# tbuckworth/train-procgen-pytorch

Hardware: AMD Instinct MI355X
Metric: env steps/sec (whole node), coinrun hard-500 IMPALA-CNN PPO (higher is better)
Workload: dtype bf16

## Files before the change

include/mi355ppo.h:

```cpp
#ifndef MI355PPO_H
#define MI355PPO_H
#include <stddef.h>
#include <stdint.h>
#ifdef __cplusplus
extern "C" {
#endif

typedef struct mi_ctx mi_ctx;

enum { MI_ARCH_IMPALA = 0, MI_ARCH_MLP = 1 };

typedef struct mi_config {
    int32_t arch;
    int32_t n_steps;
    int32_t n_envs;
    int32_t n_actions;
    int32_t obs_dim;
    int32_t mlp_depth;
    int32_t mlp_width;
    int32_t out_dim;
    int32_t max_batch;
    int32_t device;
    int32_t precision;
    int32_t value_from_logits;
// ... 20 lines not shown
int mi_copy_params(mi_ctx* dst, mi_ctx* src);
int mi_get_grads(mi_ctx* ctx, float* flat, int64_t n);
int mi_set_adam_state(mi_ctx* ctx, const float* exp_avg, const float* exp_avg_sq, int64_t n);
int mi_get_adam_state(mi_ctx* ctx, float* exp_avg, float* exp_avg_sq, int64_t n);

int mi_put_obs(mi_ctx* ctx, int32_t t, const void* obs, size_t bytes);
int mi_get_obs(mi_ctx* ctx, int32_t t, void* obs, size_t bytes);
int mi_put_step(mi_ctx* ctx, int32_t t, const float* rew, const float* done);
int mi_put_policy_outputs(mi_ctx* ctx, int32_t t, const int32_t* act, const float* logp, const float* value);
enum { MI_F_REW = 0, MI_F_DONE, MI_F_VALUE, MI_F_LOGP, MI_F_ADV, MI_F_RET, MI_F_ACT };
int mi_read_field(mi_ctx* ctx, int32_t field, float* out, int64_t n);
int mi_write_field(mi_ctx* ctx, int32_t field, const float* in, int64_t n);

int mi_policy_step(mi_ctx* ctx, int32_t t, uint64_t seed, const float* u,
                   int64_t* act_out, float* logp_out, float* value_out);

int mi_rollout_step(mi_ctx* ctx, int32_t t, const float* rew_prev, const float* done_prev, uint64_t seed, const float* u,
                    int64_t* act_out, float* logp_out, float* value_out);

int mi_rollout_groups(mi_ctx* ctx, int32_t n_groups);
int mi_rollout_submit(mi_ctx* ctx, int32_t t, int32_t group, const void* frames, size_t bytes, const float* rew_prev,
                      const float* done_prev, uint64_t seed, const float* u);
int mi_rollout_wait(mi_ctx* ctx, int32_t group, int64_t* act_out, float* logp_out, float* value_out);

int mi_predict_staged(mi_ctx* ctx, const void* obs, size_t bytes, uint64_t seed, uint64_t counter, const float* u,
                      int64_t* act_out, float* logp_out, float* value_out);
int mi_value_saliency(mi_ctx* ctx, const void* obs, size_t bytes, uint64_t seed, uint64_t counter, const float* u,
                      int64_t* act_out, float* logp_out, float* value_out, float* grad_out);
int mi_commit_staged(mi_ctx* ctx, int32_t t);

int mi_set_gru(mi_ctx* ctx, const float* w_ih, const float* w_hh, const float* b_ih, const float* b_hh);
int mi_rec_state(mi_ctx* ctx, const float* hidden , const float* done );
int mi_get_hidden(mi_ctx* ctx, float* hidden );
int mi_rec_begin(mi_ctx* ctx, const float* hidden , const float* done );
int mi_get_hidden_ring(mi_ctx* ctx, int32_t t0, int32_t t1, float* out );
int mi_forward_rec(mi_ctx* ctx, const void* obs, float* logp_all, float* value, float* hidden_out);

int mi_forward(mi_ctx* ctx, const void* obs, int32_t n, float* logp_all, float* value, float* feat);

int mi_compute_estimates(mi_ctx* ctx, float gamma, float lmbda, int32_t use_gae, int32_t normalize_adv);
int mi_adv_stats(mi_ctx* ctx, double stats3[3]);
int mi_adv_apply(mi_ctx* ctx, const double stats3[3]);

int mi_minibatch(mi_ctx* ctx, const int64_t* idx, int32_t n_idx, int32_t n_global, const mi_hparams* hp);
int mi_minibatch_multi(mi_ctx* ctx, const int64_t* idx, int32_t n_idx, const int32_t* seg_n, int32_t n_seg, int32_t n_global,
                       const mi_hparams* hp);
// ... 45 lines not shown
const char* mi_profile_class_name(int32_t class_id);

int mi_op_conv3x3(mi_ctx* ctx, int32_t mode , int32_t cin, int32_t cout, int32_t hw, int32_t n,
                  const void* in, int32_t in_is_u8, int32_t relu_in, const float* w_ref ,
                  const float* bias, const float* res, const float* mask, const float* dout,
                  float* out , float* dbias_out);
int mi_op_resblock(mi_ctx* ctx, int32_t mode, int32_t ch, int32_t hw, int32_t n, const float* x, const float* w1, const float* b1,
                   const float* w2, const float* b2, const float* a_fwd, const float* x_fwd, float* out_a, float* out_y);
int mi_op_maxpool(mi_ctx* ctx, int32_t mode , int32_t n, int32_t hw, int32_t c,
                  const float* in, const float* dout, float* out);
int mi_op_gemm(mi_ctx* ctx, int32_t M, int32_t N, int32_t K, const float* A, int64_t sam, int64_t sak,
               const float* B, int64_t sbk, int64_t sbn, float* C);
int mi_op_fc_bf16(mi_ctx* ctx, int32_t mode, int32_t n, int32_t D, const float* x, const float* W, const float* b, const float* dy,
                  float* out, float* out_b);
int mi_selftest_mfma(mi_ctx* ctx, float* max_err);
int mi_debug_read(mi_ctx* ctx, int32_t which, int32_t n, float* out);
int mi_debug_philox(mi_ctx* ctx, const uint32_t* ctr_key6, int32_t n, uint32_t* out4, float* u_out);
int mi_debug_gru_step(mi_ctx* ctx, int32_t n, int32_t H, const float* x, const float* h, const float* done, const float* w_ih,
                      const float* w_hh, const float* b_ih, const float* b_hh, float* h_out, float* h_copy);
int mi_debug_gru_seq(mi_ctx* ctx, int32_t T, int32_t n, int32_t H, const float* x, const float* h0, const float* mask, const float* w_ih,
                     const float* w_hh, const float* b_ih, const float* b_hh, const float* dOut, float* out_h, float* dX, float* dW_ih,
                     float* dW_hh, float* db_ih, float* db_hh);
int mi_debug_step_latency(mi_ctx* ctx, int32_t t, int32_t iters, int32_t mode, float* us_out);
int mi_debug_flags(mi_ctx* ctx, int32_t flags);

#ifdef __cplusplus
}
#endif
#endif
```

scratch/ro_timeline4.py:

```python
import csv, glob, sys, collections
f = glob.glob(sys.argv[1] + "/**/*kernel_trace.csv", recursive=True)[0]
rows = list(csv.DictReader(open(f)))
key = "Stream_Id" if "Stream_Id" in rows[0] else "Queue_Id"
by = collections.defaultdict(list)
for r in rows:
    by[r[key]].append(r)
streams = [(k, v) for k, v in by.items() if sum(1 for r in v if r["Kernel_Name"].startswith("heads_sample")) > 200]
print("streams with a rollout chain:", [(k, len(v)) for k, v in streams], "key", key)
k, v = streams[0]
v.sort(key=lambda r: int(r["Start_Timestamp"]))
idx = [i for i, r in enumerate(v) if r["Kernel_Name"].startswith("heads_sample")]
a, b = idx[-150], idx[-149]
base = int(v[a]["End_Timestamp"])
for r in v[a + 1:b + 1]:
    s, e = int(r["Start_Timestamp"]), int(r["End_Timestamp"])
    print(f"{(s - base) / 1e3:8.1f} us +{(e - s) / 1e3:7.1f}  {r['Kernel_Name'][:70]}")
dur, gap, cnt = collections.Counter(), collections.Counter(), collections.Counter()
for i in range(idx[-201] + 1, idx[-1] + 1):
    r, p = v[i], v[i - 1]
    n = r["Kernel_Name"][:40]
    dur[n] += (int(r["End_Timestamp"]) - int(r["Start_Timestamp"])) / 1e3
    gap[n] += (int(r["Start_Timestamp"]) - int(p["End_Timestamp"])) / 1e3
    cnt[n] += 1
print("kernel                                     n    avg_us   avg_gap_before_us")
for n in cnt:
    print(f"{n:40s} {cnt[n]:5d} {dur[n] / cnt[n]:8.1f} {gap[n] / cnt[n]:8.1f}")
print("step period us", (int(v[idx[-1]]["End_Timestamp"]) - int(v[idx[-201]]["End_Timestamp"])) / 200 / 1e3)
```

train-procgen-pytorch_amd/csrc/engine.hip:

```cpp
#include "engine_ctx.h"

thread_local std::string g_err;
thread_local hipStream_t tl_stream = nullptr;
thread_local float* tl_ws = nullptr;
thread_local size_t tl_ws_floats = 0;
const char* mi_last_error(void) { return g_err.c_str(); }

#define NCCLC(x)                                                                                         \
    do {                                                                                                 \
        ncclResult_t r_ = (x);                                                                           \
        if (r_ != ncclSuccess) return fail(-5, std::string(#x) + ": " + ncclGetErrorString(r_) + " @" + std::to_string(__LINE__)); \
    } while (0)

extern "C" int mi_comm_destroy(mi_ctx* c);
static void prof_harvest(mi_ctx* c);
static const char* kProfNames[PC_COUNT] = {
    "conv_fwd_3_16_64", "conv_fwd_16_16_32", "conv_fwd_16_32_32", "conv_fwd_32_32_16", "conv_fwd_32_32_8",
    "conv_dgrad_3_16_64(unused)", "conv_dgrad_16_16_32", "conv_dgrad_16_32_32", "conv_dgrad_32_32_16", "conv_dgrad_32_32_8",
    "conv_wgrad_3_16_64", "conv_wgrad_16_16_32", "conv_wgrad_16_32_32", "conv_wgrad_32_32_16", "conv_wgrad_32_32_8",
    "maxpool_fwd", "maxpool_bwd", "gemm", "slab_reduce",
    "resblock_fwd_(unused)", "resblock_fwd_16_16_32", "resblock_fwd_(unused)", "resblock_fwd_32_32_16", "resblock_fwd_32_32_8",
    "resblock_dgrad_(unused)", "resblock_dgrad_16_16_32", "resblock_dgrad_(unused)", "resblock_dgrad_32_32_16", "resblock_dgrad_32_32_8"};
struct GroupJob { int t; const void* frames; size_t bytes; bool pull; bool have_rd, last; const float* u; unsigned long long seed; unsigned ticket; };
struct GroupWorker {
    std::thread th; std::mutex mu; std::condition_variable cv;
    std::atomic<unsigned> posted{0}, done{0}; std::atomic<bool> sleeping{false}, quit{false};
    GroupJob job{}; int rc = 0; std::string err;
};

static inline char* obs_stage(mi_ctx* c) { return c->stage_frames ? (char*)c->stage_frames : (char*)c->stage_obs; }
struct GemmWs { float* p; size_t floats; };
static inline GemmWs gemm_ws(mi_ctx* c) { return tl_ws ? GemmWs{tl_ws, tl_ws_floats} : GemmWs{c->gemm_ws, c->gemm_ws_floats}; }
static hipStream_t side_stream(mi_ctx* c) {
    hipStream_t ss = (c->n_groups > 0 && c->gs[0]) ? c->gs[0] : c->side_stream;
    if (!ss) { hipStreamCreateWithFlags(&c->side_stream, hipStreamNonBlocking); ss = c->side_stream; }
    return ss;
}
static int64_t gru_count(const mi_ctx* c) { return 2 * (int64_t)3 * c->H * c->H + 2 * (int64_t)3 * c->H; }
struct GruTensor { float* p; size_t off, len; };
struct GruTensors { GruTensor t[4]; };
static inline GruTensors gru_tensors(mi_ctx* c) {
    const size_t H = c->H, W = 3 * H * H, B = 3 * H;
    return GruTensors{{{c->gru_wih, 0, W}, {c->gru_whh, W, W}, {c->gru_bih, 2 * W, B}, {c->gru_bhh, 2 * W + B, B}}};
}

static void add_tensor(mi_ctx* c, const std::string& name, int64_t n, int kind, int co, int ci, int64_t& ref, int64_t dev) {
    TensorDesc t{name, ref, dev, n, kind, co, ci};
    c->tensors.push_back(t);
    ref += n;
}

std::string net_err_take(mi_ctx* c) { std::lock_guard<std::mutex> lk(c->net_err_mu); std::string m; m.swap(c->net_err); return m; }
void net_err_set(mi_ctx* c, const std::string& m) { std::lock_guard<std::mutex> lk(c->net_err_mu); if (c->net_err.empty()) c->net_err = m; }

static void build_impala_layout(mi_ctx* c) {
// ... 86 lines not shown
}
static int download_flat(mi_ctx* c, const float* dbuf, float* flat, int64_t n) {
    ARG(n == c->n_params, "flat vector length != mi_param_count"); JOIN(c);
    std::vector<float> tmp(n);
    HIPC(hipMemcpyAsync(tmp.data(), dbuf, n * sizeof(float), hipMemcpyDeviceToHost, c->stream));
    HIPC(hipStreamSynchronize(c->stream));
    for (auto& t : c->tensors) to_ref_layout(t, tmp.data() + t.dev_off, flat + t.ref_off);
    return 0;
}

int mi_create(const mi_config* cfg, mi_ctx** out) {
    ARG(cfg && out, "null cfg/out");
    ARG(cfg->arch == MI_ARCH_IMPALA || cfg->arch == MI_ARCH_MLP, "arch");
    ARG(cfg->n_actions >= 1 && cfg->n_actions <= 16, "n_actions must be in [1,16]");
    ARG(cfg->n_steps >= 1 && cfg->n_envs >= 1 && cfg->max_batch >= 1, "n_steps/n_envs/max_batch");
    ARG(cfg->precision == 0 || cfg->precision == 1, "precision must be 0 (fp32) or 1 (bf16 activations)");
    ARG(cfg->value_from_logits == 0 || cfg->value_from_logits == 1, "value_from_logits must be 0 (fc_value head) or 1 (logsumexp of the logits)");
    if (cfg->arch == MI_ARCH_MLP) ARG(cfg->obs_dim >= 1 && cfg->mlp_depth >= 2 && cfg->mlp_width >= 1 && cfg->out_dim >= 1, "mlp dims");
    if (cfg->arch == MI_ARCH_IMPALA)
        ARG(cfg->out_dim == 0 || (cfg->out_dim >= 64 && cfg->out_dim <= 512 && cfg->out_dim % 64 == 0),
            "impala out_dim (output_dim) must be a multiple of 64 in [64, 512]");
    int ndev = 0;
    if (hipGetDeviceCount(&ndev) != hipSuccess || ndev == 0) return fail(-3, "no HIP device: the MI355X library has no CPU fallback");
    HIPC(hipSetDevice(cfg->device));
    mi_ctx* c = new mi_ctx();
    c->cfg = *cfg;
    c->T = cfg->n_steps; c->E = cfg->n_envs; c->A = cfg->n_actions;
    c->H = (cfg->arch == MI_ARCH_IMPALA && cfg->out_dim == 0) ? 256 : cfg->out_dim;
    c->NB = cfg->max_batch < cfg->n_envs ? cfg->n_envs : cfg->max_batch;
    c->bf = (cfg->arch == MI_ARCH_IMPALA) && cfg->precision == 1;
    c->lse = cfg->value_from_logits;
    c->es = c->bf ? 2.0 : 4.0;
    if (cfg->stream) { c->stream = (hipStream_t)cfg->stream; c->own_stream = false; }
    else { HIPC(hipStreamCreateWithFlags(&c->stream, hipStreamNonBlocking)); c->own_stream = true; }
    HIPC(hipEventCreateWithFlags(&c->ev_side_fork, hipEventDisableTiming)); HIPC(hipEventCreateWithFlags(&c->ev_side_join, hipEventDisableTiming));
    c->side_stream = nullptr; c->side_on = true; c->side.armed = false;
    if (cfg->arch == MI_ARCH_IMPALA) build_impala_layout(c); else build_mlp_layout(c);
    if (cfg->arch == MI_ARCH_IMPALA && !impala_regions_ok(c)) { delete c; return fail(-1, "internal: parameter layout does not split at embedder.fc.weight"); }

    const int64_t P = c->n_params, T = c->T, E = c->E, NB = c->NB;
    HIPC(dalloc(&c->params, P)); HIPC(dalloc(&c->grads, P)); HIPC(dalloc(&c->adam_m, P)); HIPC(dalloc(&c->adam_v, P));
    HIPC(dalloc(&c->rew, T * E)); HIPC(dalloc(&c->done, T * E)); HIPC(dalloc(&c->logp, T * E));
    HIPC(dalloc(&c->adv, T * E)); HIPC(dalloc(&c->ret, T * E)); HIPC(dalloc(&c->value, (T + 1) * E));
    HIPC(dalloc(&c->act, T * E)); HIPC(dalloc(&c->adv_stats, 4));
    c->frames = nullptr; c->obsf = nullptr; c->stage_frames = nullptr; c->stage_obs = nullptr;
    if (cfg->arch == MI_ARCH_IMPALA) {
// ... 107 lines not shown
    }
    c->gru_x = c->gru_dg = nullptr; c->sal_keep_x = c->bwd_from_dfeat = false;
    c->gru_on = false; c->gru_wih = c->gru_whh = c->gru_bih = c->gru_bhh = c->h_state = c->h_masked = c->gru_gi = c->gru_gh = c->d_done = nullptr;
    c->h_ring = c->h_rec_stage = nullptr; c->ev_rec = nullptr; for (bool& b : c->g_rec_ok) b = false;
    c->gru_train = c->rec_last = false; c->gru_g = c->gru_m = c->gru_v = nullptr; c->gru_sumsq = nullptr;
    c->rec_x = c->rec_gi = c->rec_sv = c->rec_dgi = c->rec_dgh = c->rec_hm = c->rec_mask = c->rec_h0 = nullptr;
    HIPC(hipDeviceSynchronize());
    *out = c;
    return 0;
}

int mi_destroy(mi_ctx* c) {
    if (!c) return 0;
    mi_comm_destroy(c);
    for (int g = 0; g < mi_ctx::MAX_GROUPS; ++g)
        if (c->gw[g]) {
            GroupWorker* w = c->gw[g];
            w->quit.store(true); { std::lock_guard<std::mutex> lk(w->mu); } w->cv.notify_one();
            w->th.join(); delete w; c->gw[g] = nullptr;
        }
    for (int g = 0; g < mi_ctx::MAX_GROUPS; ++g) if (c->gs[g]) hipStreamSynchronize(c->gs[g]);
    prof_harvest(c);
    hipStreamSynchronize(c->stream);
    for (int g = 0; g < mi_ctx::MAX_GROUPS; ++g) if (c->gs[g]) { hipStreamDestroy(c->gs[g]); hipEventDestroy(c->ev_fork[g]); hipEventDestroy(c->ev_join[g]); }
    for (hipEvent_t e : c->prof.pool) hipEventDestroy(e);
    float* fl[] = {c->params, c->grads, c->adam_m, c->adam_v, c->rew, c->done, c->logp, c->adv, c->ret, c->value, c->obsf,
                   c->feat, c->dfeat, c->hout, c->dY, c->GC, c->GP[0], c->GP[1], c->GP[2], c->slabs, c->gemm_ws, c->col_ws,
                   c->fs_scratch, c->fs_val, c->lut, c->stage_obs, c->loss_partial, c->loss_stats, c->loss_log, c->gnorm,
                   c->d_u, c->d_lp};
    for (float* p : fl) if (p) hipFree(p);
    if (c->cfg.arch == MI_ARCH_IMPALA)
        for (int b = 0; b < 3; ++b) { Block& k = c->blk[b]; hipFree(k.C); hipFree(k.PI); hipFree(k.P0); hipFree(k.A1); hipFree(k.P1); hipFree(k.A2); hipFree(k.P2); }
    for (float* p : c->mlp_act) if (p) hipFree(p);
    if (c->frames) hipFree(c->frames);
    if (c->stage_frames) hipFree(c->stage_frames);
    hipFree(c->s_act); hipFree(c->s_logp); hipFree(c->s_val);
    if (c->d_val) hipFree(c->d_val);
    if (c->fc_wp) hipFree(c->fc_wp); if (c->fc_wt) hipFree(c->fc_wt);
    if (c->banks) hipFree(c->banks); if (c->d_bank_desc) hipFree(c->d_bank_desc); if (c->c1_bank) hipFree(c->c1_bank);
    hipFree(c->stats_ring); hipFree(c->fs_ring); hipFree(c->fs_parts); if (c->d_slab_desc) hipFree(c->d_slab_desc); if (c->sal_dc) hipFree(c->sal_dc); if (c->sal_dx) hipFree(c->sal_dx); hipFree(c->d_pack); hipFree(c->d_rd); hipHostFree(c->h_pack); hipHostFree(c->h_rd); hipFree(c->d_done_ctr); if (c->side_stream) hipStreamDestroy(c->side_stream); hipEventDestroy(c->ev_side_fork); hipEventDestroy(c->ev_side_join); hipHostFree(c->h_flag);
    { float* gr[] = {c->gru_wih, c->gru_whh, c->gru_bih, c->gru_bhh, c->h_state, c->h_masked, c->gru_gi, c->gru_gh, c->d_done, c->gru_x, c->gru_dg}; for (float* q : gr) if (q) hipFree(q); }
    if (c->h_ring) hipFree(c->h_ring); if (c->h_rec_stage) hipHostFree(c->h_rec_stage); if (c->ev_rec) hipEventDestroy(c->ev_rec);
    { float* gt[] = {c->gru_g, c->gru_m, c->gru_v, c->rec_x, c->rec_gi, c->rec_sv, c->rec_dgi, c->rec_dgh, c->rec_hm, c->rec_mask, c->rec_h0}; for (float* q : gt) if (q) hipFree(q); }
    if (c->gru_sumsq) hipFree(c->gru_sumsq);
    hipFree(c->act); hipFree(c->adv_stats); hipFree(c->d_idx); hipFree(c->sumsq);
    if (c->fs_colmax) hipFree(c->fs_colmax); if (c->fs_arg) hipFree(c->fs_arg);
    if (c->fs_keys) hipFree(c->fs_keys); if (c->fs_keys_local) hipFree(c->fs_keys_local); if (c->d_gpos) hipFree(c->d_gpos); if (c->h_gpos) hipHostFree(c->h_gpos);
// ... 739 lines not shown
        while (w->posted.load(std::memory_order_acquire) == seen && !w->quit.load()) {
            if (++spins < 40000) __builtin_ia32_pause();
            else {
                std::unique_lock<std::mutex> lk(w->mu);
                w->sleeping.store(true);
                w->cv.wait_for(lk, std::chrono::milliseconds(50), [&] { return w->posted.load() != seen || w->quit.load(); });
                w->sleeping.store(false);
                spins = 0;
            }
        }
        if (w->quit.load()) return;
        seen = w->posted.load(std::memory_order_acquire);
        w->rc = group_issue(c, g, w->job);
        if (w->rc) w->err = g_err;
        w->done.store(seen, std::memory_order_release);
    }
}

int mi_rollout_groups(mi_ctx* c, int32_t n_groups) {
    ARG(c, "null"); ARG(n_groups >= 1 && n_groups <= mi_ctx::MAX_GROUPS, "1 .. 4 groups");
    ARG(c->E % n_groups == 0, "n_envs must be divisible by the number of groups");
    for (int g = 0; g < c->n_groups; ++g) ARG(!c->g_busy[g], "a group step is still in flight: mi_rollout_wait it first");
    JOIN(c);
    for (int g = 0; g < n_groups; ++g)
        if (!c->gs[g]) {
            HIPC(hipStreamCreateWithFlags(&c->gs[g], hipStreamNonBlocking));
            HIPC(hipEventCreateWithFlags(&c->ev_fork[g], hipEventDisableTiming));
            HIPC(hipEventCreateWithFlags(&c->ev_join[g], hipEventDisableTiming));
            c->gw[g] = new GroupWorker();
            c->gw[g]->th = std::thread(group_worker_main, c, g);
        }
    c->n_groups = n_groups;
    return 0;
}

int mi_rollout_submit(mi_ctx* c, int32_t t, int32_t g, const void* frames, size_t bytes, const float* rew_prev, const float* done_prev,
                      uint64_t seed, const float* u) {
    ARG(c, "null"); ARG(t >= 0 && t <= c->T, "t out of range"); ARG(g >= 0 && g < c->n_groups, "group out of range");
    ARG(c->gs[g], "call mi_rollout_groups first"); ARG(!c->g_busy[g], "this group's previous step has not been waited for");
    ARG(c->pending_n < 0, "a multirank minibatch is pending");
    const int E = c->E, ng = E / c->n_groups, e0 = g * ng;
    ARG(!frames || bytes == (size_t)ng * c->obs_bytes_per_env, "frames byte count != (E / groups) * bytes_per_env");
    if (rew_prev || done_prev) ARG(rew_prev && done_prev && t >= 1, "rew_prev/done_prev come together and belong to step t-1");
    if (c->gru_on) {
        ARG(c->h_ring && (t > 0 || c->g_rec_ok[g]), "recurrent rollout: call mi_rec_begin before the groups' first step (t == 0) of every rollout");
        if (t == 0) c->g_rec_ok[g] = false;
    }
    GroupWorker* w = c->gw[g];
    worker_drain(w);
    if (!c->g_forked[g]) {
        fc_refresh(c);
        HIPC(hipEventRecord(c->ev_fork[g], c->main_stream));
        HIPC(hipStreamWaitEvent(c->gs[g], c->ev_fork[g], 0));
        c->g_forked[g] = true;
    }
// ... 605 lines not shown
```

train-procgen-pytorch_amd/csrc/engine_ctx.h:

```cpp
#pragma once
#include "common.h"
#include "../../include/mi355ppo.h"
#include <rccl/rccl.h>
#include <math.h>
#include <stdio.h>
#include <string.h>
#include <string>
#include <unordered_map>
#include <vector>
#include <atomic>
#include <chrono>
#include <condition_variable>
#include <mutex>
#include <thread>

#pragma clang diagnostic ignored "-Wc++20-designator"
#define MI_INTERNAL __attribute__((visibility("hidden")))

MI_INTERNAL extern thread_local std::string g_err;
MI_INTERNAL extern thread_local hipStream_t tl_stream;
MI_INTERNAL extern thread_local float* tl_ws;
MI_INTERNAL extern thread_local size_t tl_ws_floats;
#define CUR(c) (tl_stream ? tl_stream : (c)->stream)
static inline int fail(int code, const std::string& msg) { g_err = msg; return code; }
// ... 69 lines not shown
    unsigned short* lut16;
    uint8_t* stage_frames; float* stage_obs;
    int32_t* d_idx;
    float *loss_partial, *loss_stats, *loss_log; int log_count, log_cap;
    double* fs_parts;
    float *stats_ring, *fs_ring; LossArgs ring_args;
    double* sumsq; float* gnorm;
    float* d_u; float* d_lp;
    unsigned short* banks; BankDesc* d_bank_desc; int n_banks;
    unsigned short* c1_bank;
    unsigned short *fc_wp, *fc_wt;
    bool fc_packed_valid;
    float *d_pack, *h_pack, *h_rd, *d_rd;
    unsigned *d_done_ctr, *h_flag, roll_ticket;
    int32_t* s_act; float *s_logp, *s_val; bool staged_valid;
    bool gru_on; float *gru_wih, *gru_whh, *gru_bih, *gru_bhh, *h_state, *h_masked, *gru_gi, *gru_gh, *d_done;
    float *gru_x, *gru_dg; bool sal_keep_x, bwd_from_dfeat;
    static constexpr int IDX_RING = 32;
    int32_t* h_idx_ring[IDX_RING]; hipEvent_t idx_ev[IDX_RING]; bool idx_used[IDX_RING]; int idx_next, idx_ev_deferred;
    float* h_f; int32_t* h_i; size_t h_f_floats;
    int multirank;
    LossArgs pending; int pending_n;
    static constexpr int MAX_GROUPS = 4;
    int n_groups; hipStream_t main_stream, gs[MAX_GROUPS]; hipEvent_t ev_fork[MAX_GROUPS], ev_join[MAX_GROUPS];
    bool g_forked[MAX_GROUPS], g_busy[MAX_GROUPS], g_last[MAX_GROUPS], g_dirty[MAX_GROUPS]; unsigned g_ticket[MAX_GROUPS]; bool groups_live;
    struct GroupWorker* gw[MAX_GROUPS];
    std::atomic<int64_t> copy_slot_ns{0}; double copy_rate_bytes_per_us;
    std::unordered_map<const void*, bool> pull_ok; bool no_pull;
    hipStream_t side_stream; hipEvent_t ev_side_fork, ev_side_join;
    bool side_on;
    struct SideJob { bool armed; LossArgs a; SegTab st; int mode; float* ring; float* fsr; float* log; } side;
    bool rollout_tail;
    float *fs_colmax, fs_grad_coef; int *fs_arg, fs_G;
    long long *fs_keys, *fs_keys_local; int32_t *d_gpos, *h_gpos; int gpos_n; bool fs_global_pending, fs_global_apply;
    ncclComm_t comm, comm_grad; int comm_world, comm_rank; hipStream_t comm_stream; hipEvent_t ev_ar_ready, ev_ar_done;
    bool ar_armed, ar_issued, ar_inflight; double* adv_all;
    std::string net_err; std::mutex net_err_mu;
    float *h_ring, *h_rec_stage; hipEvent_t ev_rec; bool g_rec_ok[MAX_GROUPS];
    bool gru_train, rec_last; float *gru_g, *gru_m, *gru_v; double* gru_sumsq;
    float *rec_x, *rec_gi, *rec_sv, *rec_dgi, *rec_dgh, *rec_hm, *rec_mask, *rec_h0;
};

static inline char* obs_ring(mi_ctx* c) { return c->frames ? (char*)c->frames : (char*)c->obsf; }

MI_INTERNAL std::string net_err_take(mi_ctx* c);
MI_INTERNAL void net_err_set(mi_ctx* c, const std::string& m);
MI_INTERNAL int join_groups(mi_ctx* c);
// ... 18 lines not shown
```

train-procgen-pytorch_amd/csrc/engine_ops.hip:

```cpp
#include "engine_ctx.h"

static int shape_of(int cin, int cout, int hw, ConvShape* s) {
    for (int k = 0; k < CS_COUNT; ++k) {
        int a, b, h; conv_shape_dims((ConvShape)k, &a, &b, &h);
        if (a == cin && b == cout && h == hw) { *s = (ConvShape)k; return 0; }
    }
    return fail(-1, "unsupported conv shape");
}

std::vector<uint16_t> host_to_bf16(const float* x, size_t n) {
    std::vector<uint16_t> o(n);
    for (size_t k = 0; k < n; ++k) { uint32_t u; memcpy(&u, x + k, 4); o[k] = (uint16_t)((u + 0x7FFFu + ((u >> 16) & 1u)) >> 16); }
    return o;
}
static void host_from_bf16(const uint16_t* h, float* x, size_t n) {
    for (size_t k = 0; k < n; ++k) { const uint32_t u = ((uint32_t)h[k]) << 16; memcpy(x + k, &u, 4); }
}
struct OpMem {
    static constexpr size_t GUARD = 64 * 1024;
    static constexpr int CANARY = 0xA5;
    struct Band { std::string name; unsigned char* p; size_t bytes; bool rezero; };
    const char* hook; hipStream_t st;
    std::vector<void*> owned;
    std::vector<Band> bands;
// ... 352 lines not shown
    HIPC(hipStreamSynchronize(c->stream));
    hipGraph_t graph = nullptr; hipGraphExec_t exec = nullptr;
    if (mode == 1) {
        HIPC(hipStreamBeginCapture(c->stream, hipStreamCaptureModeThreadLocal));
        issue();
        HIPC(hipStreamEndCapture(c->stream, &graph));
        HIPC(hipGraphInstantiate(&exec, graph, nullptr, nullptr, 0));
        HIPC(hipGraphLaunch(exec, c->stream)); HIPC(hipStreamSynchronize(c->stream));
    }
    const auto t0 = std::chrono::steady_clock::now();
    for (int k = 0; k < iters; ++k) {
        if (mode == 1) HIPC(hipGraphLaunch(exec, c->stream)); else issue();
        HIPC(hipStreamSynchronize(c->stream));
    }
    const auto t1 = std::chrono::steady_clock::now();
    *us_out = (float)(std::chrono::duration_cast<std::chrono::nanoseconds>(t1 - t0).count() / 1e3 / iters);
    if (exec) hipGraphExecDestroy(exec);
    if (graph) hipGraphDestroy(graph);
    c->prof.on = prof_on;
    HIPC(hipGetLastError()); NETCHK(c);
    return 0;
}

int mi_debug_read(mi_ctx* c, int32_t which, int32_t n, float* out) {
    ARG(c && out, "null"); JOIN(c); ARG(n >= 1 && n <= c->NB, "n must be in [1, max_batch]");
    if (which == 100 || which == 101 || which == 102) {
        ARG(which == 100 || c->rec_last, "which = 101 / 102: only after mi_minibatch_rec");
        const float* srcp = which == 102 ? c->dfeat : (which == 100 && c->rec_last) ? c->rec_x : c->feat;
        HIPC(hipMemcpyAsync(out, srcp, (size_t)n * c->H * 4, hipMemcpyDeviceToHost, c->stream));
        HIPC(hipStreamSynchronize(c->stream));
        return 0;
    }
    ARG(c->cfg.arch == MI_ARCH_IMPALA && which >= 0 && which < 24 && (which & 7) <= 5, "which");
    const Block& k = c->blk[which >> 3];
    const size_t pe = (size_t)n * (k.hin / 2) * (k.hin / 2) * k.cout;
    HIPC(hipStreamSynchronize(c->stream));
    if ((which & 7) == 5) {
        std::vector<uint8_t> h(pe);
        HIPC(hipMemcpy(h.data(), k.PI, pe, hipMemcpyDeviceToHost));
        for (size_t i = 0; i < pe; ++i) out[i] = (float)h[i];
        return 0;
    }
    const float* src[5] = {k.P0, k.A1, k.P1, k.A2, k.P2};
    return download_act(c, src[which & 7], out, pe);
}

// ... 117 lines not shown
```

train-procgen-pytorch_amd/mi355/engine.py:

```python
import ctypes as C
import os

import numpy as np

_HERE = os.path.dirname(os.path.abspath(__file__))
_LIB = None

ARCH_IMPALA, ARCH_MLP = 0, 1
F_REW, F_DONE, F_VALUE, F_LOGP, F_ADV, F_RET, F_ACT = range(7)
PTR_GRADS, PTR_LOSS_STATS, PTR_PARAMS, PTR_STATS_RING, PTR_FS_KEYS = 0, 1, 2, 3, 4
LOSS_FIELDS = ("pi_loss", "value_loss", "entropy", "x_ent", "total", "fs", "marg", "_pad")


class EngineError(RuntimeError):
    pass


class _Config(C.Structure):
    _fields_ = [("arch", C.c_int32), ("n_steps", C.c_int32), ("n_envs", C.c_int32), ("n_actions", C.c_int32),
                ("obs_dim", C.c_int32), ("mlp_depth", C.c_int32), ("mlp_width", C.c_int32), ("out_dim", C.c_int32),
                ("max_batch", C.c_int32), ("device", C.c_int32), ("precision", C.c_int32), ("value_from_logits", C.c_int32),
                ("reserved", C.c_int32 * 4),
                ("stream", C.c_void_p)]


class _HParams(C.Structure):
    _fields_ = [(n, C.c_float) for n in ("eps_clip", "value_coef", "entropy_coef", "x_entropy_coef",
                                         "entropy_multiplier", "fs_coef")]


def lib_path():
    return os.path.join(_HERE, "libmi355ppo.so")


EXPORTS = ("mi_last_error mi_create mi_destroy mi_sync mi_host_alloc mi_host_free mi_host_register mi_host_unregister mi_param_count mi_set_params "
           "mi_get_params mi_copy_params mi_get_grads mi_set_adam_state mi_get_adam_state mi_put_obs mi_get_obs mi_put_step "
           "mi_put_policy_outputs mi_read_field mi_write_field mi_policy_step mi_rollout_step mi_rollout_groups mi_rollout_submit mi_rollout_wait mi_predict_staged mi_value_saliency mi_commit_staged mi_set_gru mi_rec_state mi_get_hidden mi_rec_begin mi_get_hidden_ring mi_forward_rec mi_forward mi_compute_estimates "
           "mi_adv_stats mi_adv_apply mi_minibatch mi_minibatch_multi mi_optimizer_step mi_loss_log_read mi_device_ptr "
           "mi_set_multirank mi_minibatch_finish mi_loss_log_finalize mi_profile_enable mi_profile_read mi_profile_class_name mi_op_conv3x3 mi_op_resblock mi_op_maxpool mi_op_gemm mi_op_fc_bf16 mi_selftest_mfma mi_debug_read mi_debug_flags mi_comm_unique_id mi_comm_init mi_comm_destroy mi_allreduce_arm mi_allreduce_grads mi_allreduce_buffer mi_adv_normalize_global mi_minibatch_positions mi_debug_philox mi_debug_gru_step mi_debug_step_latency "
           "mi_gru_train mi_minibatch_rec mi_get_gru mi_get_gru_grads mi_get_gru_adam_state mi_set_gru_adam_state mi_debug_gru_seq "
           "mi_sae_create mi_sae_destroy mi_sae_param_count mi_sae_set_params mi_sae_get_params mi_sae_get_grads mi_sae_set_adam_state mi_sae_get_adam_state mi_sae_put_ring "
           "mi_sae_get_hidden mi_sae_get_logits mi_sae_step mi_sae_minibatch mi_sae_probe_minibatch mi_sae_optimizer_step mi_sae_debug_forward").split()


def load_library():
    global _LIB
    if _LIB is not None:
        return _LIB
    path = lib_path()
    if not os.path.exists(path):
        raise EngineError(f"{path} not found: build it with `make -C train-procgen-pytorch_amd/csrc` "
                          "(python __graft_entry__.py build).  There is no CPU fallback.")
    lib = C.CDLL(path)
    lib.mi_last_error.restype = C.c_char_p
    lib.mi_param_count.restype = C.c_int64
    lib.mi_sae_param_count.restype = C.c_int64
    lib.mi_host_alloc.restype = C.c_void_p
    lib.mi_host_alloc.argtypes = [C.c_size_t]
    lib.mi_host_free.argtypes = [C.c_void_p]
    lib.mi_host_free.restype = None
    lib.mi_profile_class_name.restype = C.c_char_p
    lib.mi_host_register.argtypes = [C.c_void_p, C.c_size_t]
# ... 164 lines not shown
        self._chk(self.lib.mi_policy_step(self._ctx, C.c_int32(t), C.c_uint64(seed), _fp(u), _fp(act), _fp(logp), _fp(val)))
        return act, logp, val

    def rollout_step(self, t, rew_prev=None, done_prev=None, seed=0, u=None):
        u = None if u is None else _f32(u)
        if rew_prev is not None and (not isinstance(rew_prev, np.ndarray) or rew_prev.dtype != np.float32 or not rew_prev.flags.c_contiguous):
            rew_prev = _f32(rew_prev)
        if done_prev is not None and (not isinstance(done_prev, np.ndarray) or done_prev.dtype != np.float32 or not done_prev.flags.c_contiguous):
            done_prev = _f32(done_prev)
        E = self.E
        out = np.empty(4 * E, np.float32)
        p = out.__array_interface__['data'][0]
        rc = self.lib.mi_rollout_step(self._ctx, t, None if rew_prev is None else rew_prev.__array_interface__['data'][0],
                                      None if done_prev is None else done_prev.__array_interface__['data'][0], seed,
                                      None if u is None else u.__array_interface__['data'][0], p, p + 8 * E, p + 12 * E)
        if rc:
            self._chk(rc)
        return out[:2 * E].view(np.int64), out[2 * E:3 * E], out[3 * E:]

    def rollout_groups(self, n_groups):
        self._chk(self.lib.mi_rollout_groups(self._ctx, C.c_int32(n_groups)))
        self.n_groups = n_groups

    def rollout_submit(self, t, group, frames=None, rew_prev=None, done_prev=None, seed=0, u=None):
        addr = lambda a: None if a is None else a.__array_interface__['data'][0]
        if rew_prev is not None and (rew_prev.dtype != np.float32 or not rew_prev.flags.c_contiguous):
            rew_prev = _f32(rew_prev)
        if done_prev is not None and (done_prev.dtype != np.float32 or not done_prev.flags.c_contiguous):
            done_prev = _f32(done_prev)
        u = None if u is None else _f32(u)
        if frames is not None and not frames.flags.c_contiguous:
            raise EngineError("rollout_submit needs a contiguous (pinned) frame buffer")
        rc = self.lib.mi_rollout_submit(self._ctx, t, group, addr(frames), 0 if frames is None else frames.nbytes, addr(rew_prev), addr(done_prev), seed, addr(u))
        if rc:
            self._chk(rc)
        self._keep_alive = (frames, rew_prev, done_prev, u)

    def rollout_wait(self, group):
        n = self.E // getattr(self, "n_groups", 1)
        out = np.empty(4 * n, np.float32)
        p = out.__array_interface__['data'][0]
        rc = self.lib.mi_rollout_wait(self._ctx, group, p, p + 8 * n, p + 12 * n)
        if rc:
            self._chk(rc)
        return out[:2 * n].view(np.int64), out[2 * n:3 * n], out[3 * n:]

# ... 377 lines not shown
        g = np.ascontiguousarray(gpos, dtype=np.int32)
        self._chk(self.lib.mi_minibatch_positions(self._ctx, g.ctypes.data_as(C.c_void_p), C.c_int32(g.size)))

    def debug_philox(self, ctr_key6):
        a = np.ascontiguousarray(ctr_key6, dtype=np.uint32).reshape(-1, 6)
        out, u = np.empty((a.shape[0], 4), np.uint32), np.empty(a.shape[0], np.float32)
        self._chk(self.lib.mi_debug_philox(self._ctx, _fp(a), C.c_int32(a.shape[0]), _fp(out), _fp(u)))
        return out, u

    def debug_gru_step(self, x, h, done, w_ih, w_hh, b_ih, b_hh, with_copy=False):
        x, h = _f32(x), _f32(h)
        n, H = x.shape
        a = [_f32(v) for v in (done, w_ih, w_hh, b_ih, b_hh)]
        out = np.empty((n, H), np.float32)
        cp = np.empty((n, H), np.float32) if with_copy else None
        self._chk(self.lib.mi_debug_gru_step(self._ctx, C.c_int32(n), C.c_int32(H), _fp(x), _fp(h), *[_fp(v) for v in a], _fp(out), _fp(cp)))
        return (out, cp) if with_copy else out

    def debug_step_latency(self, t, iters=200, graph=False):
        us = C.c_float(0)
        self._chk(self.lib.mi_debug_step_latency(self._ctx, C.c_int32(t), C.c_int32(iters), C.c_int32(int(graph)), C.byref(us)))
        return us.value

    def debug_flags(self, flags):
        self._chk(self.lib.mi_debug_flags(self._ctx, C.c_int32(flags)))

    def selftest_mfma(self):
        e = C.c_float(0)
        self._chk(self.lib.mi_selftest_mfma(self._ctx, C.byref(e)))
        return e.value
```

Before: 599,400.

## Share high-priority group streams across contexts via a per-device lane registry

Rollout group streams are no longer created per context. They are borrowed from a per-device registry of up to four streams created at the highest stream priority, with the least-used lane handed out first. The goal is to cut the number of hardware queues that per-group streams from many contexts on one device are spread across, and to give rollout chains priority over other work. The trade-off is that contexts sharing a lane serialize their rollout kernels on it. Debug helpers are also added to report lane priority and stream identity and to time a sleep kernel across lanes.

```diff
diff --git a/include/mi355ppo.h b/include/mi355ppo.h
--- a/include/mi355ppo.h
+++ b/include/mi355ppo.h
@@ -66,6 +66,7 @@
 int mi_rollout_submit(mi_ctx* ctx, int32_t t, int32_t group, const void* frames, size_t bytes, const float* rew_prev,
                       const float* done_prev, uint64_t seed, const float* u);
 int mi_rollout_wait(mi_ctx* ctx, int32_t group, int64_t* act_out, float* logp_out, float* value_out);
+int mi_rollout_lane_info(mi_ctx* ctx, int32_t* n, int32_t* prio , uint64_t* stream_id );
 
 int mi_predict_staged(mi_ctx* ctx, const void* obs, size_t bytes, uint64_t seed, uint64_t counter, const float* u,
                       int64_t* act_out, float* logp_out, float* value_out);
@@ -157,6 +158,7 @@
                      const float* w_hh, const float* b_ih, const float* b_hh, const float* dOut, float* out_h, float* dX, float* dW_ih,
                      float* dW_hh, float* db_ih, float* db_hh);
 int mi_debug_step_latency(mi_ctx* ctx, int32_t t, int32_t iters, int32_t mode, float* us_out);
+int mi_debug_lane_probe(mi_ctx* ctx, int32_t mask, int32_t iters, float* usec);
 int mi_debug_flags(mi_ctx* ctx, int32_t flags);
 
 #ifdef __cplusplus
diff --git a/scratch/lane_queues.py b/scratch/lane_queues.py
--- /dev/null
+++ b/scratch/lane_queues.py
@@ -0,0 +1,49 @@
+import csv, glob, sys, collections
+f = glob.glob(sys.argv[1] + "/**/*kernel_trace.csv", recursive=True)[0]
+rows = list(csv.DictReader(open(f)))
+print("columns:", list(rows[0].keys()))
+print("kernels:", len(rows))
+if "Stream_Id" not in rows[0]:
+    q = collections.Counter(r["Queue_Id"] for r in rows if ("heads_sample" in r["Kernel_Name"]))
+    print("no Stream_Id column; heads_sample kernels per Queue_Id:", dict(q))
+    sys.exit(0)
+by = collections.defaultdict(list)
+for r in rows:
+    by[r["Stream_Id"]].append(r)
+print("| Stream_Id | kernels | heads_sample | Queue_Id: kernels |")
+print("|---|---|---|---|")
+chains = []
+for k, v in sorted(by.items(), key=lambda kv: int(kv[0])):
+    hs = sum(1 for r in v if ("heads_sample" in r["Kernel_Name"]))
+    q = collections.Counter(r["Queue_Id"] for r in v)
+    print(f"| {k} | {len(v)} | {hs} | {dict(q)} |")
+    if hs > 200:
+        chains.append(k)
+print("streams with a rollout chain:", chains)
+byq = collections.defaultdict(list)
+for r in rows:
+    if r["Stream_Id"] in chains:
+        byq[r["Queue_Id"]].append(r)
+tot = other = tight = 0
+waits = []
+for q, v in byq.items():
+    v.sort(key=lambda r: int(r["Start_Timestamp"]))
+    for i in range(1, len(v)):
+        r, p = v[i], v[i - 1]
+        if "conv1_pool_fwd" not in r["Kernel_Name"]:
+            continue
+        tot += 1
+        if p["Stream_Id"] != r["Stream_Id"] and ("heads_sample" in p["Kernel_Name"]):
+            other += 1
+            gap = (int(r["Start_Timestamp"]) - int(p["End_Timestamp"])) / 1e3
+            waits.append(gap)
+            if gap < 10.0:
+                tight += 1
+print(f"conv1_pool_fwd launches of the chains: {tot}; preceded on their queue by ANOTHER chain's heads_sample: {other}; "
+      f"of those started within 10 us of its end: {tight}")
+if waits:
+    waits.sort()
+    print(f"gap after the other chain's heads_sample, us: median {waits[len(waits) // 2]:.1f}, p10 {waits[len(waits) // 10]:.1f}, p90 {waits[9 * len(waits) // 10]:.1f}")
+for k in chains:
+    v = sorted((r for r in by[k] if ("heads_sample" in r["Kernel_Name"])), key=lambda r: int(r["End_Timestamp"]))
+    print(f"stream {k}: step period {(int(v[-1]['End_Timestamp']) - int(v[-201]['End_Timestamp'])) / 200 / 1e3:.1f} us")
diff --git a/scratch/ro_timeline4.py b/scratch/ro_timeline4.py
--- a/scratch/ro_timeline4.py
+++ b/scratch/ro_timeline4.py
@@ -5,11 +5,11 @@
 by = collections.defaultdict(list)
 for r in rows:
     by[r[key]].append(r)
-streams = [(k, v) for k, v in by.items() if sum(1 for r in v if r["Kernel_Name"].startswith("heads_sample")) > 200]
+streams = [(k, v) for k, v in by.items() if sum(1 for r in v if "heads_sample" in r["Kernel_Name"]) > 200]
 print("streams with a rollout chain:", [(k, len(v)) for k, v in streams], "key", key)
 k, v = streams[0]
 v.sort(key=lambda r: int(r["Start_Timestamp"]))
-idx = [i for i, r in enumerate(v) if r["Kernel_Name"].startswith("heads_sample")]
+idx = [i for i, r in enumerate(v) if "heads_sample" in r["Kernel_Name"]]
 a, b = idx[-150], idx[-149]
 base = int(v[a]["End_Timestamp"])
 for r in v[a + 1:b + 1]:
diff --git a/train-procgen-pytorch_amd/csrc/engine.hip b/train-procgen-pytorch_amd/csrc/engine.hip
--- a/train-procgen-pytorch_amd/csrc/engine.hip
+++ b/train-procgen-pytorch_amd/csrc/engine.hip
@@ -1,4 +1,5 @@
 #include "engine_ctx.h"
+#include "lanes.h"
 
 thread_local std::string g_err;
 thread_local hipStream_t tl_stream = nullptr;
@@ -31,6 +32,21 @@
 static inline char* obs_stage(mi_ctx* c) { return c->stage_frames ? (char*)c->stage_frames : (char*)c->stage_obs; }
 struct GemmWs { float* p; size_t floats; };
 static inline GemmWs gemm_ws(mi_ctx* c) { return tl_ws ? GemmWs{tl_ws, tl_ws_floats} : GemmWs{c->gemm_ws, c->gemm_ws_floats}; }
+static constexpr int MAX_LANE_DEVICES = 64;
+static LaneRegistry* const g_lanes = new LaneRegistry[MAX_LANE_DEVICES];
+static void* lane_make(int device, int, int* prio) {
+    int dev0 = 0, least = 0, greatest = 0;
+    hipStream_t s = nullptr;
+    if (hipGetDevice(&dev0) != hipSuccess || hipSetDevice(device) != hipSuccess) return nullptr;
+    const bool ok = hipDeviceGetStreamPriorityRange(&least, &greatest) == hipSuccess &&
+                    hipStreamCreateWithPriority(&s, hipStreamNonBlocking, greatest) == hipSuccess &&
+                    hipStreamGetPriority(s, prio) == hipSuccess;
+    hipSetDevice(dev0);
+    if (!ok && s) { hipStreamDestroy(s); s = nullptr; }
+    return s;
+}
+static void lane_drop(void* s) { hipStreamDestroy((hipStream_t)s); }
+
 static hipStream_t side_stream(mi_ctx* c) {
     hipStream_t ss = (c->n_groups > 0 && c->gs[0]) ? c->gs[0] : c->side_stream;
     if (!ss) { hipStreamCreateWithFlags(&c->side_stream, hipStreamNonBlocking); ss = c->side_stream; }
@@ -163,6 +179,7 @@
             "impala out_dim (output_dim) must be a multiple of 64 in [64, 512]");
     int ndev = 0;
     if (hipGetDeviceCount(&ndev) != hipSuccess || ndev == 0) return fail(-3, "no HIP device: the MI355X library has no CPU fallback");
+    ARG(cfg->device >= 0 && cfg->device < ndev && cfg->device < MAX_LANE_DEVICES, "device");
     HIPC(hipSetDevice(cfg->device));
     mi_ctx* c = new mi_ctx();
     c->cfg = *cfg;
@@ -316,7 +333,8 @@
     for (int g = 0; g < mi_ctx::MAX_GROUPS; ++g) if (c->gs[g]) hipStreamSynchronize(c->gs[g]);
     prof_harvest(c);
     hipStreamSynchronize(c->stream);
-    for (int g = 0; g < mi_ctx::MAX_GROUPS; ++g) if (c->gs[g]) { hipStreamDestroy(c->gs[g]); hipEventDestroy(c->ev_fork[g]); hipEventDestroy(c->ev_join[g]); }
+    for (int g = 0; g < mi_ctx::MAX_GROUPS; ++g) if (c->gs[g]) { hipEventDestroy(c->ev_fork[g]); hipEventDestroy(c->ev_join[g]); c->gs[g] = nullptr; }
+    g_lanes[c->cfg.device].give_back(c, lane_drop);
     for (hipEvent_t e : c->prof.pool) hipEventDestroy(e);
     float* fl[] = {c->params, c->grads, c->adam_m, c->adam_v, c->rew, c->done, c->logp, c->adv, c->ret, c->value, c->obsf,
                    c->feat, c->dfeat, c->hout, c->dY, c->GC, c->GP[0], c->GP[1], c->GP[2], c->slabs, c->gemm_ws, c->col_ws,
@@ -1102,15 +1120,26 @@
     ARG(c->E % n_groups == 0, "n_envs must be divisible by the number of groups");
     for (int g = 0; g < c->n_groups; ++g) ARG(!c->g_busy[g], "a group step is still in flight: mi_rollout_wait it first");
     JOIN(c);
+    void* lane[mi_ctx::MAX_GROUPS]; int prio[mi_ctx::MAX_GROUPS];
+    const int have = [&] { int k = 0; while (k < mi_ctx::MAX_GROUPS && c->gs[k]) ++k; return k; }();
+    if (n_groups > have && !g_lanes[c->cfg.device].borrow(c, n_groups, c->cfg.device, lane_make, lane, prio))
+        return fail(-2, "no stream for an env group (hipStreamCreateWithPriority failed)");
     for (int g = 0; g < n_groups; ++g)
         if (!c->gs[g]) {
-            HIPC(hipStreamCreateWithFlags(&c->gs[g], hipStreamNonBlocking));
+            c->gs[g] = (hipStream_t)lane[g]; c->gs_prio[g] = prio[g];
             HIPC(hipEventCreateWithFlags(&c->ev_fork[g], hipEventDisableTiming));
             HIPC(hipEventCreateWithFlags(&c->ev_join[g], hipEventDisableTiming));
             c->gw[g] = new GroupWorker();
             c->gw[g]->th = std::thread(group_worker_main, c, g);
         }
     c->n_groups = n_groups;
+    return 0;
+}
+
+int mi_rollout_lane_info(mi_ctx* c, int32_t* n, int32_t* prio, uint64_t* stream_id) {
+    ARG(c && n && prio && stream_id, "null");
+    *n = 0;
+    for (int g = 0; g < c->n_groups && c->gs[g]; ++g) { prio[g] = c->gs_prio[g]; stream_id[g] = (uint64_t)(uintptr_t)c->gs[g]; *n = g + 1; }
     return 0;
 }
 
diff --git a/train-procgen-pytorch_amd/csrc/engine_ctx.h b/train-procgen-pytorch_amd/csrc/engine_ctx.h
--- a/train-procgen-pytorch_amd/csrc/engine_ctx.h
+++ b/train-procgen-pytorch_amd/csrc/engine_ctx.h
@@ -115,7 +115,7 @@
     int multirank;
     LossArgs pending; int pending_n;
     static constexpr int MAX_GROUPS = 4;
-    int n_groups; hipStream_t main_stream, gs[MAX_GROUPS]; hipEvent_t ev_fork[MAX_GROUPS], ev_join[MAX_GROUPS];
+    int n_groups; hipStream_t main_stream, gs[MAX_GROUPS]; int gs_prio[MAX_GROUPS]; hipEvent_t ev_fork[MAX_GROUPS], ev_join[MAX_GROUPS];
     bool g_forked[MAX_GROUPS], g_busy[MAX_GROUPS], g_last[MAX_GROUPS], g_dirty[MAX_GROUPS]; unsigned g_ticket[MAX_GROUPS]; bool groups_live;
     struct GroupWorker* gw[MAX_GROUPS];
     std::atomic<int64_t> copy_slot_ns{0}; double copy_rate_bytes_per_us;
diff --git a/train-procgen-pytorch_amd/csrc/engine_ops.hip b/train-procgen-pytorch_amd/csrc/engine_ops.hip
--- a/train-procgen-pytorch_amd/csrc/engine_ops.hip
+++ b/train-procgen-pytorch_amd/csrc/engine_ops.hip
@@ -398,6 +398,24 @@
     return 0;
 }
 
+__global__ void __launch_bounds__(64) lane_probe_kernel(int iters) {
+    for (int i = 0; i < iters; ++i) __builtin_amdgcn_s_sleep(127);
+}
+int mi_debug_lane_probe(mi_ctx* c, int32_t mask, int32_t iters, float* usec) {
+    ARG(c && usec, "null"); JOIN(c);
+    ARG(mask > 0 && mask < (1 << c->n_groups) && iters >= 1, "mask (bits of this context's groups) / iters");
+    for (int g = 0; g < c->n_groups; ++g) ARG(c->gs[g] && !c->g_busy[g], "call mi_rollout_groups first; no group step in flight");
+    if (iters > 4096) iters = 4096;
+    for (int g = 0; g < c->n_groups; ++g) if (mask >> g & 1) HIPC(hipStreamSynchronize(c->gs[g]));
+    const auto t0 = std::chrono::steady_clock::now();
+    for (int g = 0; g < c->n_groups; ++g) if (mask >> g & 1) lane_probe_kernel<<<1, 64, 0, c->gs[g]>>>(iters);
+    for (int g = 0; g < c->n_groups; ++g) if (mask >> g & 1) HIPC(hipStreamSynchronize(c->gs[g]));
+    const auto t1 = std::chrono::steady_clock::now();
+    HIPC(hipGetLastError());
+    *usec = (float)(std::chrono::duration_cast<std::chrono::nanoseconds>(t1 - t0).count() / 1e3);
+    return 0;
+}
+
 int mi_debug_read(mi_ctx* c, int32_t which, int32_t n, float* out) {
     ARG(c && out, "null"); JOIN(c); ARG(n >= 1 && n <= c->NB, "n must be in [1, max_batch]");
     if (which == 100 || which == 101 || which == 102) {
diff --git a/train-procgen-pytorch_amd/csrc/lanes.h b/train-procgen-pytorch_amd/csrc/lanes.h
--- /dev/null
+++ b/train-procgen-pytorch_amd/csrc/lanes.h
@@ -0,0 +1,55 @@
+#pragma once
+#include <mutex>
+#include <utility>
+#include <vector>
+
+struct LaneRegistry {
+    static constexpr int MAX_LANES = 4;
+    typedef void* (*MakeFn)(int key, int lane, int* prio);
+    typedef void (*DropFn)(void* stream);
+
+    bool borrow(const void* owner, int want, int key, MakeFn make, void** out, int* prio) {
+        std::lock_guard<std::mutex> lk(mu_);
+        if (want < 1 || want > MAX_LANES) return false;
+        Holder* h = find(owner);
+        if (!h) { holders_.push_back(Holder{owner, {}}); h = &holders_.back(); }
+        while ((int)h->lanes.size() < want) {
+            int best = -1;
+            for (int l = 0; l < MAX_LANES; ++l) {
+                bool held = false;
+                for (int x : h->lanes) held = held || x == l;
+                if (!held && (best < 0 || lane_[l].users < lane_[best].users)) best = l;
+            }
+            Lane& L = lane_[best];
+            if (!L.stream) {
+                L.stream = make(key, best, &L.prio);
+                if (!L.stream) { if (h->lanes.empty()) forget(owner); return false; }
+            }
+            ++L.users;
+            h->lanes.push_back(best);
+        }
+        for (int k = 0; k < want; ++k) { out[k] = lane_[h->lanes[k]].stream; if (prio) prio[k] = lane_[h->lanes[k]].prio; }
+        return true;
+    }
+    void give_back(const void* owner, DropFn drop) {
+        std::lock_guard<std::mutex> lk(mu_);
+        Holder* h = find(owner);
+        if (!h) return;
+        for (int l : h->lanes) --lane_[l].users;
+        forget(owner);
+        if (!holders_.empty()) return;
+        for (Lane& L : lane_) { if (L.stream) drop(L.stream); L = Lane{}; }
+    }
+    int users(int lane) { std::lock_guard<std::mutex> lk(mu_); return lane_[lane].users; }
+    int live_streams() { std::lock_guard<std::mutex> lk(mu_); int n = 0; for (const Lane& L : lane_) n += L.stream != nullptr; return n; }
+    int lane_of(const void* owner, int k) { std::lock_guard<std::mutex> lk(mu_); Holder* h = find(owner); return h && k < (int)h->lanes.size() ? h->lanes[k] : -1; }
+
+private:
+    struct Lane { void* stream = nullptr; int prio = 0; int users = 0; };
+    struct Holder { const void* owner; std::vector<int> lanes; };
+    Holder* find(const void* owner) { for (Holder& h : holders_) if (h.owner == owner) return &h; return nullptr; }
+    void forget(const void* owner) { for (size_t i = 0; i < holders_.size(); ++i) if (holders_[i].owner == owner) { holders_.erase(holders_.begin() + i); return; } }
+    std::mutex mu_;
+    Lane lane_[MAX_LANES];
+    std::vector<Holder> holders_;
+};
diff --git a/train-procgen-pytorch_amd/mi355/engine.py b/train-procgen-pytorch_amd/mi355/engine.py
--- a/train-procgen-pytorch_amd/mi355/engine.py
+++ b/train-procgen-pytorch_amd/mi355/engine.py
@@ -35,9 +35,9 @@
 
 EXPORTS = ("mi_last_error mi_create mi_destroy mi_sync mi_host_alloc mi_host_free mi_host_register mi_host_unregister mi_param_count mi_set_params "
            "mi_get_params mi_copy_params mi_get_grads mi_set_adam_state mi_get_adam_state mi_put_obs mi_get_obs mi_put_step "
-           "mi_put_policy_outputs mi_read_field mi_write_field mi_policy_step mi_rollout_step mi_rollout_groups mi_rollout_submit mi_rollout_wait mi_predict_staged mi_value_saliency mi_commit_staged mi_set_gru mi_rec_state mi_get_hidden mi_rec_begin mi_get_hidden_ring mi_forward_rec mi_forward mi_compute_estimates "
+           "mi_put_policy_outputs mi_read_field mi_write_field mi_policy_step mi_rollout_step mi_rollout_groups mi_rollout_lane_info mi_rollout_submit mi_rollout_wait mi_predict_staged mi_value_saliency mi_commit_staged mi_set_gru mi_rec_state mi_get_hidden mi_rec_begin mi_get_hidden_ring mi_forward_rec mi_forward mi_compute_estimates "
            "mi_adv_stats mi_adv_apply mi_minibatch mi_minibatch_multi mi_optimizer_step mi_loss_log_read mi_device_ptr "
-           "mi_set_multirank mi_minibatch_finish mi_loss_log_finalize mi_profile_enable mi_profile_read mi_profile_class_name mi_op_conv3x3 mi_op_resblock mi_op_maxpool mi_op_gemm mi_op_fc_bf16 mi_selftest_mfma mi_debug_read mi_debug_flags mi_comm_unique_id mi_comm_init mi_comm_destroy mi_allreduce_arm mi_allreduce_grads mi_allreduce_buffer mi_adv_normalize_global mi_minibatch_positions mi_debug_philox mi_debug_gru_step mi_debug_step_latency "
+           "mi_set_multirank mi_minibatch_finish mi_loss_log_finalize mi_profile_enable mi_profile_read mi_profile_class_name mi_op_conv3x3 mi_op_resblock mi_op_maxpool mi_op_gemm mi_op_fc_bf16 mi_selftest_mfma mi_debug_read mi_debug_flags mi_comm_unique_id mi_comm_init mi_comm_destroy mi_allreduce_arm mi_allreduce_grads mi_allreduce_buffer mi_adv_normalize_global mi_minibatch_positions mi_debug_philox mi_debug_gru_step mi_debug_step_latency mi_debug_lane_probe "
            "mi_gru_train mi_minibatch_rec mi_get_gru mi_get_gru_grads mi_get_gru_adam_state mi_set_gru_adam_state mi_debug_gru_seq "
            "mi_sae_create mi_sae_destroy mi_sae_param_count mi_sae_set_params mi_sae_get_params mi_sae_get_grads mi_sae_set_adam_state mi_sae_get_adam_state mi_sae_put_ring "
            "mi_sae_get_hidden mi_sae_get_logits mi_sae_step mi_sae_minibatch mi_sae_probe_minibatch mi_sae_optimizer_step mi_sae_debug_forward").split()
@@ -248,6 +248,11 @@
         self._chk(self.lib.mi_rollout_groups(self._ctx, C.c_int32(n_groups)))
         self.n_groups = n_groups
 
+    def lane_info(self):
+        n, prio, sid = C.c_int32(0), (C.c_int32 * 4)(), (C.c_uint64 * 4)()
+        self._chk(self.lib.mi_rollout_lane_info(self._ctx, C.byref(n), prio, sid))
+        return [(int(prio[g]), int(sid[g])) for g in range(n.value)]
+
     def rollout_submit(self, t, group, frames=None, rew_prev=None, done_prev=None, seed=0, u=None):
         addr = lambda a: None if a is None else a.__array_interface__['data'][0]
         if rew_prev is not None and (rew_prev.dtype != np.float32 or not rew_prev.flags.c_contiguous):
@@ -671,6 +676,11 @@
         self._chk(self.lib.mi_debug_step_latency(self._ctx, C.c_int32(t), C.c_int32(iters), C.c_int32(int(graph)), C.byref(us)))
         return us.value
 
+    def debug_lane_probe(self, mask, iters):
+        us = C.c_float(0)
+        self._chk(self.lib.mi_debug_lane_probe(self._ctx, C.c_int32(mask), C.c_int32(iters), C.byref(us)))
+        return us.value
+
     def debug_flags(self, flags):
         self._chk(self.lib.mi_debug_flags(self._ctx, C.c_int32(flags)))
 
```

Measured after the change: 714,000 (median of 6 runs). +19.1%, better.
